# PhantomSDR/PhantomSDR

Measured on AMD Instinct MI355X. Metric: ingest MSamples/s + concurrent audio clients at 2^20-pt FFT, higher is better.
Workload: dtype f32

## Files before the change

phantomsdr_amd/csrc/demod.h:

```cpp
#pragma once
#include <hip/hip_runtime.h>
#include <stdint.h>

#include "butterfly.h"
#include "quantize.h"
#include "types.h"

namespace psdr {



struct DemodArgs {
    const cf *spec;
    size_t spec_stride;
    SpecLayout lay;
    int is_real;
    int n;
    int nframes;
    int max_batch;
    unsigned long long first_frame_num;
    const ClientParams *clients;
    const cf *Wn;
    int nstages;
    int radix[PSDR_MAX_STAGES];
    const int4 *stage_tab;
    cf *ypost;
    float *pwr;
    cf *gscratch;
    int lds_mode;
    float *audio;
    int *nan_flags;
    float *real_prev;
    cf *bb_tail;
    cf *bb_last;
    int slots;
    unsigned *ssb_mark;
    unsigned mark_epoch;
    int replay;
    const int4 *notch_man;
    const int4 *notch_auto;
};
__device__ __forceinline__ bool not_finite(float v) { return !(fabsf(v) <= 3.402823466e38f); }

__device__ __forceinline__ bool flip_frame(unsigned long long frame_num, int m_idx, int is_real) {
    return (frame_num % 2 == 1) && ((m_idx % 2 == 0 && !is_real) || (m_idx % 2 == 1 && is_real));
}
__device__ __forceinline__ float frame_sign(const DemodArgs &a, const ClientParams &cp, int f) {
    return flip_frame(a.first_frame_num + (unsigned long long)f, cp.m_floor, a.is_real) ? -1.f : 1.f;
}

__device__ __forceinline__ void wave_lds_sync() { asm volatile("s_waitcnt lgkmcnt(0)" ::: "memory"); }
__device__ __forceinline__ float wave_sum(float v) {
#pragma unroll
    for (int d = 32; d > 0; d >>= 1) v += __shfl_xor(v, d, 64);
    return v;
}
__device__ __forceinline__ cf *stage_twiddles(const DemodArgs &a, unsigned char *smem, int n) {
    cf *Wn = reinterpret_cast<cf *>(smem);
    for (int i = threadIdx.x; i < n; i += blockDim.x) Wn[i] = a.Wn[i];
    __syncthreads();
    return Wn;
}
__device__ __forceinline__ bool wave_chain(int nact, int F, int K, int &ci, int &f0, int &f1) {
// ... 298 lines not shown
        t = x[1], x[1] = x[3], x[3] = t;
        t = x[2], x[2] = x[6], x[6] = t;
        t = x[5], x[5] = x[7], x[7] = t;
    } else {
        static_assert(R == 10, "butterflies with literal roots: 5, 8, 9, 10");
        idft5(x[0], x[2], x[4], x[6], x[8]);
        idft5(x[1], x[3], x[5], x[7], x[9]);
        const cf w1 = make_float2(0.80901699437494742410f, 0.58778525229247312917f);
        const cf w2 = make_float2(0.30901699437494742410f, 0.95105651629515357212f);
        const cf w3 = make_float2(-0.30901699437494742410f, 0.95105651629515357212f);
        const cf w4 = make_float2(-0.80901699437494742410f, 0.58778525229247312917f);
        cf o1, o2, o3, o4;
        cmul_pair(o1, x[3], w1, o2, x[5], w2);
        cmul_pair(o3, x[7], w3, o4, x[9], w4);
        const cf e0 = x[0], e1 = x[2], e2 = x[4], e3 = x[6], e4 = x[8], o0 = x[1];
        x[0] = cadd(e0, o0), x[5] = csub(e0, o0);
        x[1] = cadd(e1, o1), x[6] = csub(e1, o1);
        x[2] = cadd(e2, o2), x[7] = csub(e2, o2);
        x[3] = cadd(e3, o3), x[8] = csub(e3, o3);
        x[4] = cadd(e4, o4), x[9] = csub(e4, o4);
    }
}

template <int N, int R, int PP>
__device__ __forceinline__ void idft_stage_fixed(cf *buf, const cf *Wn, int lane) {
    constexpr int TLEN = N / R, ROUNDS = (TLEN + 63) / 64, STEP = N / (PP * R);
    constexpr bool RAGGED = (TLEN % 64) != 0;
    cf x[ROUNDS][R];
    int jo[ROUNDS];
#pragma unroll
    for (int rr = 0; rr < ROUNDS; rr++) {
        const int i = lane + 64 * rr;
        if (!RAGGED || rr + 1 < ROUNDS || i < TLEN) {
            const int k = PP == 1 ? 0 : i % PP;
            jo[rr] = (i - k) * R + k;
            x[rr][0] = buf[i];
#pragma unroll
            for (int q = 1; q < R; q++) {
                const cf v = buf[i + q * TLEN];
                if (PP > 1)
                    x[rr][q] = cmul(v, Wn[q * k * STEP]);
                else
                    x[rr][q] = v;
            }
        }
    }
    asm volatile("" ::: "memory");
#pragma unroll
    for (int rr = 0; rr < ROUNDS; rr++) {
        const int i = lane + 64 * rr;
        if (!RAGGED || rr + 1 < ROUNDS || i < TLEN) {
            cf *o = buf + jo[rr];
            idft_bfly<R>(x[rr]);
#pragma unroll
            for (int s = 0; s < R; s++) o[s * PP] = x[rr][s];
        }
    }
}

template <int N>
__device__ __forceinline__ void idft_load_slice(const DemodArgs &a, const ClientParams &cp, const Notches &nz, int f, int lane, cf (&sv)[(N + 63) / 64]) {
    const int len = cp.r - cp.l;
    const cf *S = a.spec + (size_t)f * a.spec_stride;
#pragma unroll
    for (int u = 0; u < (N + 63) / 64; u++) {
        const int t = lane + 64 * u;
        sv[u] = t < len && !notched(nz, cp, t) ? S[a.lay.pos(cp.l + t)] : make_float2(0.f, 0.f);
    }
}
template <int N, int HO>
__device__ __forceinline__ void idft_slice_offsets(const DemodArgs &a, const ClientParams &cp, int lane, unsigned (&so)[HO]) {
    const int len = cp.r - cp.l;
#pragma unroll
    for (int u = 0; u < HO; u++) {
        const int t = lane + 64 * u;
        so[u] = t < len ? (unsigned)a.lay.pos(cp.l + t) : 0u;
    }
}
template <int N, int HO, bool NZ = true>
__device__ __forceinline__ void idft_load_slice_at(const DemodArgs &a, const ClientParams &cp, const Notches &nz, int f, const unsigned (&so)[HO], int lane, cf (&sv)[(N + 63) / 64]) {
    const int len = cp.r - cp.l;
    const cf *S = a.spec + (size_t)f * a.spec_stride;
#pragma unroll
    for (int u = 0; u < (N + 63) / 64; u++) {
        const int t = lane + 64 * u;
        const bool in = t < len && !(NZ && notched(nz, cp, t));
        if (u < HO)
            sv[u] = in ? S[so[u]] : make_float2(0.f, 0.f);
        else
            sv[u] = in ? S[a.lay.pos(cp.l + t)] : make_float2(0.f, 0.f);
    }
}
template <int N, int R0, int R1, int R2>
__device__ __forceinline__ float idft_slice_fixed(const ClientParams &cp, const cf (&sv)[(N + 63) / 64], cf *buf, const cf *Wn, int lane);
template <int N, int R0, int R1, int R2>
__device__ __forceinline__ float idft_item_fixed(const DemodArgs &a, const ClientParams &cp, int f, cf *buf, const cf *Wn, int lane) {
    cf sv[(N + 63) / 64];
    idft_load_slice<N>(a, cp, notch_load(a, cp.slot), f, lane, sv);
    return idft_slice_fixed<N, R0, R1, R2>(cp, sv, buf, Wn, lane);
}
template <int N, int R0, int R1, int R2>
__device__ __forceinline__ float idft_slice_fixed(const ClientParams &cp, const cf (&sv)[(N + 63) / 64], cf *buf, const cf *Wn, int lane) {
    const int len = cp.r - cp.l;
    const int m = cp.m_floor - cp.l;
    constexpr int NR = (N + 63) / 64;
#pragma unroll
    for (int u = 0; u < NR; u++) {
        const int i = lane + 64 * u;
        if (i < N) buf[i] = make_float2(0.f, 0.f);
    }
    asm volatile("" ::: "memory");
    float pw = 0.f;
#pragma unroll
    for (int u = 0; u < NR; u++) {
        const int t = lane + 64 * u;
        if (t < len) {
            const cf v = sv[u];
            pw += fmaf(v.x, v.x, v.y * v.y);
            if (cp.mode < 2) {
                const int idx = cp.mode == 0 ? t - m : m - t;
                if (idx == 0 || idx == N / 2) {
                    buf[idx] = make_float2(v.x, 0.f);
                } else if (idx > 0 && idx < N / 2) {
                    buf[idx] = v;
                    buf[N - idx] = make_float2(v.x, -v.y);
                }
            } else {
                if (t >= m && t < m + N / 2) buf[t - m] = v;
                if (t >= m - N / 2 + 1 && t < m) buf[N - m + t] = v;
            }
        }
    }
    pw = wave_sum(pw);
    wave_lds_sync();
    idft_stage_fixed<N, R0, 1>(buf, Wn, lane);
    wave_lds_sync();
    idft_stage_fixed<N, R1, R0>(buf, Wn, lane);
    wave_lds_sync();
    if constexpr (R2 > 1) {
        idft_stage_fixed<N, R2, R0 * R1>(buf, Wn, lane);
        wave_lds_sync();
    }
    return pw;
}

template <int N, int R0, int R1, int R2>
#ifndef PSDR_IDFT_WPE
#define PSDR_IDFT_WPE 5
#endif
__global__ __launch_bounds__(256, PSDR_IDFT_WPE) void k_demod_idft_fixed(DemodArgs a, int nact) {
    static_assert(R0 * R1 * R2 == N, "plan");
    extern __shared__ __attribute__((aligned(16))) unsigned char smem[];
    const int lane = threadIdx.x & 63, wv = threadIdx.x >> 6;
    cf *Wn = stage_twiddles(a, smem, N);
    int ci, f, f1;
    if (!wave_chain(nact, a.nframes, 1, ci, f, f1)) return;
    const ClientParams cp = wave_uniform(a.clients[ci]);
    cf *buf = Wn + N + (size_t)wv * N;

    const float pw = idft_item_fixed<N, R0, R1, R2>(a, cp, f, buf, Wn, lane);
    if (lane == 0) a.pwr[(size_t)cp.slot * a.max_batch + f] = pw;
    constexpr int NR = (N + 63) / 64;
    const float sg = frame_sign(a, cp, f);
// ... 124 lines not shown
    const size_t srow = (size_t)cp.slot;
    if (cp.mode >= 2 || a.ssb_mark[srow] != a.mark_epoch) return;
    const cf *yp = a.ypost + (srow * a.max_batch) * n;
    const SlotState st = slot_state(a, cp, h);
    int g = -1;
    for (int f = 0; f < a.nframes; f++) {
        const cf *y = yp + (size_t)f * n;
        float *out = a.audio + (srow * a.max_batch + f) * h;
        int s_nan = 0;
        for (int j = tid; j < h; j += NT) {
            const float prev = (g < 0) ? st.rp_old[j] : yp[(size_t)g * n + h + j].x;
            const float v = y[j].x + prev;
            out[j] = v;
            if (isnan(v)) s_nan = 1;
        }
        const int dropped = __any(s_nan);
        if (tid == 0) a.nan_flags[srow * a.max_batch + f] = dropped ? 1 : 0;
        if (!dropped) g = f;
    }
    for (int j = tid; j < h; j += NT) st.rp_new[j] = (g < 0) ? st.rp_old[j] : yp[(size_t)g * n + h + j].x;
}


template <int N, int R0, int R1, int R2>
__global__ __launch_bounds__(256, N <= 512 ? PSDR_IDFT_WPE : PSDR_IDFT_WPE - 1) void k_demod_chain_fixed(DemodArgs a, int nact, int K) {
    static_assert(R0 * R1 * R2 == N, "plan");
    extern __shared__ __attribute__((aligned(16))) unsigned char smem[];
    constexpr int h = N / 2, NH = (h + 63) / 64;
    const int lane_ = threadIdx.x & 63, wv = threadIdx.x >> 6;
    cf *Wn = stage_twiddles(a, smem, N);
    const int F = a.nframes;
    int ci, f0, f1;
    if (!wave_chain(nact, F, K, ci, f0, f1)) return;
    ClientParams cp = a.clients[ci];
    if (a.replay && (cp.mode >= 2 || a.ssb_mark[cp.slot] != a.mark_epoch)) return;
    cp = wave_uniform(cp);
    cf *buf = Wn + N + (size_t)wv * N;
    const size_t srow = (size_t)cp.slot;
    const SlotState st = slot_state(a, cp, h);
    const bool ssb = cp.mode < 2;
    cf tail[NH];
    cf blast = make_float2(0.f, 0.f);
    const int fs = f0 == 0 ? 0 : (f0 - (cp.mode == 3 ? 2 : 1) > 0 ? f0 - (cp.mode == 3 ? 2 : 1) : 0);
#pragma unroll
    for (int u = 0; u < NH; u++) {
        const int j = lane_ + 64 * u;
        tail[u] = make_float2(0.f, 0.f);
        if (fs == 0 && j < h) tail[u] = ssb ? make_float2(st.rp_old[j], 0.f) : st.bt_old[j];
    }
    if (fs == 0 && cp.mode == 3) blast = a.bb_last[st.row_old];
    int bad = 0;
    if (ssb) {
#pragma unroll
        for (int u = 0; u < NH; u++) bad |= not_finite(tail[u].x) ? 1 : 0;
    }
    int f = fs;
#ifndef PSDR_DEMOD_PREFETCH
#define PSDR_DEMOD_PREFETCH 0
#endif
    constexpr int NR = (N + 63) / 64;
    cf svn[NR];
    int fpre = -1;
    constexpr int HO = NR < 3 ? NR : (N <= 512 ? 3 : 6);
    unsigned so[HO];
    idft_slice_offsets<N, HO>(a, cp, lane_, so);
    const Notches nz = notch_load(a, cp.slot);
    while (f < f1) {
        const bool emit = f >= f0;
        const int lane = opaque_lane(lane_);
        float pw;
        if (PSDR_DEMOD_PREFETCH && (N <= 512 || PSDR_DEMOD_PREFETCH > 1)) {
            cf sv[NR];
            if (f == fpre) {
#pragma unroll
                for (int u = 0; u < NR; u++) sv[u] = svn[u];
            } else {
                idft_load_slice_at<N, HO>(a, cp, nz, f, so, lane, sv);
            }
            if (f + 1 < f1) {
                idft_load_slice_at<N, HO>(a, cp, nz, f + 1, so, lane, svn);
                fpre = f + 1;
            }
            pw = idft_slice_fixed<N, R0, R1, R2>(cp, sv, buf, Wn, lane);
        } else {
            cf sv[NR];
            idft_load_slice_at<N, HO>(a, cp, nz, f, so, lane, sv);
            pw = idft_slice_fixed<N, R0, R1, R2>(cp, sv, buf, Wn, lane);
        }
        if (emit && lane == 0) a.pwr[srow * a.max_batch + f] = pw;
        const float sg = frame_sign(a, cp, f);
        float *out = a.audio + (srow * a.max_batch + f) * h;
        const bool last = (f == F - 1);
        int s_nan = 0;
        cf carry = blast;
        cf yv[NH], yn[NH];
        if (cp.mode == 0) {
#pragma unroll
            for (int u = 0; u < NH; u++) {
                const int j = lane + 64 * u;
                yv[u] = yn[u] = make_float2(0.f, 0.f);
                if (j < h) {
                    yv[u].x = __fmul_rn(buf[j].x, sg);
                    yn[u].x = __fmul_rn(buf[h + j].x, sg);
                }
            }
        } else if (cp.mode == 1) {
#pragma unroll
            for (int u = 0; u < NH; u++) {
                const int j = lane + 64 * u;
                yv[u] = yn[u] = make_float2(0.f, 0.f);
                if (j < h) {
                    yv[u].x = __fmul_rn(buf[N - 1 - j].x, sg);
                    yn[u].x = __fmul_rn(buf[N - 1 - h - j].x, sg);
                }
            }
        } else {
#pragma unroll
            for (int u = 0; u < NH; u++) {
                const int j = lane + 64 * u;
                yv[u] = yn[u] = make_float2(0.f, 0.f);
                if (j < h) {
                    const cf v0 = buf[j], v1 = buf[h + j];
                    yv[u] = make_float2(__fmul_rn(v0.x, sg), __fmul_rn(v0.y, sg));
                    yn[u] = make_float2(__fmul_rn(v1.x, sg), __fmul_rn(v1.y, sg));
                }
            }
        }
#pragma unroll
        for (int u = 0; u < NH; u++) {
            const int j = lane + 64 * u;
            const bool ok = j < h;
            const cf y = yv[u], ynext = yn[u];
            float v = 0.f;
            cf b = make_float2(0.f, 0.f);
            if (ssb) {
                v = __fadd_rn(y.x, tail[u].x);
            } else {
                b = make_float2(__fadd_rn(y.x, tail[u].x), __fadd_rn(y.y, tail[u].y));
                if (cp.mode == 2) {
                    v = sqrtf(fmaf(b.x, b.x, b.y * b.y));
                } else {
                    cf pr = make_float2(__shfl_up(b.x, 1, 64), __shfl_up(b.y, 1, 64));
                    if (lane == 0) pr = carry;
                    const float re = fmaf(b.x, pr.x, b.y * pr.y);
                    const float im = fmaf(b.x, -pr.y, b.y * pr.x);
                    v = atan2f(im, re);
                    carry = make_float2(__shfl(b.x, 63, 64), __shfl(b.y, 63, 64));
                    if (u == (h - 1) / 64) blast = make_float2(__shfl(b.x, (h - 1) & 63, 64), __shfl(b.y, (h - 1) & 63, 64));
// ... 2 lines not shown
            if (ok && isnan(v)) s_nan = 1;
            if (ok && emit) {
                out[j] = v;
                if (last && !ssb) {
                    st.bt_new[j] = ynext;
                    st.rp_new[j] = st.rp_old[j];
                    if (j == h - 1) a.bb_last[st.row_new] = b;
                }
            }
            if (!ssb) tail[u] = ynext;
        }
        const int any_nan = __any(s_nan);
        if (ssb) {
#pragma unroll
            for (int u = 0; u < NH; u++) bad |= (not_finite(yv[u].x) || not_finite(yn[u].x)) ? 1 : 0;
            if (!emit) {
                if (any_nan && f > 0) {
                    f--;
                    wave_lds_sync();
                    continue;
                }
#pragma unroll
                for (int u = 0; u < NH; u++) {
                    const int j = lane + 64 * u;
                    tail[u] = yn[u];
                    if (any_nan && j < h) tail[u] = make_float2(st.rp_old[j], 0.f);
                }
                f = f0;
                wave_lds_sync();
                continue;
            }
#pragma unroll
            for (int u = 0; u < NH; u++) {
                const int j = lane + 64 * u;
                if (!any_nan) tail[u] = yn[u];
                if (last && j < h) {
                    st.rp_new[j] = tail[u].x;
                    st.bt_new[j] = st.bt_old[j];
                }
            }
            if (last && lane == 0) a.bb_last[st.row_new] = a.bb_last[st.row_old];
        }
        if (emit && lane == 0) a.nan_flags[srow * a.max_batch + f] = any_nan ? 1 : 0;
        wave_lds_sync();
        f++;
    }
    if (ssb && !a.replay && __any(bad) && lane_ == 0) a.ssb_mark[srow] = a.mark_epoch;
}


template <int N, int R0, int R1, int R2, bool NZ>
__device__ __forceinline__ void demod_chain_iq_body(const DemodArgs &a, int nact, int K, cf *iq) {
    static_assert(R0 * R1 * R2 == N, "plan");
    extern __shared__ __attribute__((aligned(16))) unsigned char smem[];
    constexpr int h = N / 2, NH = (h + 63) / 64;
    const int lane_ = threadIdx.x & 63, wv = threadIdx.x >> 6;
    cf *Wn = stage_twiddles(a, smem, N);
    const int F = a.nframes;
    int ci, f0, f1;
    if (!wave_chain(nact, F, K, ci, f0, f1)) return;
    const ClientParams cp = wave_uniform(a.clients[ci]);
    cf *buf = Wn + N + (size_t)wv * N;
    const size_t srow = (size_t)cp.slot;
    const SlotState st = slot_state(a, cp, h);
    const int fs = f0 == 0 ? 0 : f0 - 1;
    cf tail[NH];
#pragma unroll
    for (int u = 0; u < NH; u++) {
        const int j = lane_ + 64 * u;
        tail[u] = make_float2(0.f, 0.f);
        if (fs == 0 && j < h) tail[u] = st.bt_old[j];
    }
    constexpr int NR = (N + 63) / 64;
    constexpr int HO = NR < 3 ? NR : (N <= 512 ? 3 : 6);
    unsigned so[HO];
    idft_slice_offsets<N, HO>(a, cp, lane_, so);
    for (int f = fs; f < f1; f++) {
        const bool emit = f >= f0;
        const int lane = opaque_lane(lane_);
        Notches nz{};
        if constexpr (NZ) nz = notch_load_frame(a, cp.slot);
        cf sv[NR];
        idft_load_slice_at<N, HO, NZ>(a, cp, nz, f, so, lane, sv);
        const float pw = idft_slice_fixed<N, R0, R1, R2>(cp, sv, buf, Wn, lane);
        if (emit && lane == 0) a.pwr[srow * a.max_batch + f] = pw;
        const float sg = frame_sign(a, cp, f);
        cf *out = iq + (srow * a.max_batch + f) * h;
        const bool last = (f == F - 1);
        int s_nan = 0;
#pragma unroll
        for (int u = 0; u < NH; u++) {
            const int j = lane + 64 * u;
            if (j < h) {
                const cf v0 = buf[j], v1 = buf[h + j];
                const cf y = make_float2(__fmul_rn(v0.x, sg), __fmul_rn(v0.y, sg));
                const cf ynext = make_float2(__fmul_rn(v1.x, sg), __fmul_rn(v1.y, sg));
                const cf b = make_float2(__fadd_rn(y.x, tail[u].x), __fadd_rn(y.y, tail[u].y));
                if (isnan(b.x) || isnan(b.y)) s_nan = 1;
                if (emit) {
                    out[j] = b;
                    if (last) {
                        st.bt_new[j] = ynext;
                        st.rp_new[j] = st.rp_old[j];
                        if (j == h - 1) a.bb_last[st.row_new] = b;
                    }
                }
                tail[u] = ynext;
// ... 89 lines not shown
    idft_slice_offsets<N, HO>(a, cp, lane_, so);
    const int m = cp.m_floor - cp.l;
    cf cC[NH];
#pragma unroll
    for (int u = 0; u < NH; u++) cC[u] = make_float2(0.f, 0.f);
    for (int it = 2 * fs; it < 2 * f1; it++) {
        const int f = it >> 1, pass = it & 1;
        const bool emit = f >= f0;
        const float sg = frame_sign(a, cp, f);
        float *out = a.audio + (srow * a.max_batch + f) * h;
        const bool last = (f == F - 1);
        {
            const int lane = opaque_lane(lane_);
            const Notches nz = notch_load_frame(a, cp.slot);
            cf sv[NR];
            idft_load_slice_at<N, HO>(a, cp, nz, f, so, lane, sv);
            if (pass == 0) {
#pragma unroll
                for (int u = 0; u < NR; u++) {
                    const int d = lane + 64 * u - m;
                    if (d < -sa.cutoff || d >= sa.cutoff) sv[u] = make_float2(0.f, 0.f);
                }
            }
            const float pw = idft_slice_fixed<N, R0, R1, R2>(cp, sv, buf, Wn, lane);
            if (pass == 0) {
#pragma unroll
                for (int u = 0; u < NH; u++) {
                    const int j = lane + 64 * u;
                    cC[u] = make_float2(0.f, 0.f);
                    if (j < h) {
                        const cf v0 = buf[j], v1 = buf[h + j];
                        const cf ct = ctail[j];
                        cC[u] = make_float2(__fadd_rn(__fmul_rn(v0.x, sg), ct.x), __fadd_rn(__fmul_rn(v0.y, sg), ct.y));
                        ctail[j] = make_float2(__fmul_rn(v1.x, sg), __fmul_rn(v1.y, sg));
                    }
                }
            } else {
                if (emit && lane == 0) a.pwr[srow * a.max_batch + f] = pw;
                int s_nan = 0;
                float lvl = 0.f;
                cf lag = make_float2(0.f, 0.f), ccarry = make_float2(0.f, 0.f);
#pragma unroll
                for (int u = 0; u < NH; u++) {
                    const int j = lane + 64 * u;
                    const cf c = cC[u];
                    cf pr = make_float2(__shfl_up(c.x, 1, 64), __shfl_up(c.y, 1, 64));
                    if (lane == 0) pr = ccarry;
// ... 191 lines not shown
        const cf t = ft_rot(64u * (unsigned)u * fc.step);
        wu[u] = make_float2(__int_as_float(__builtin_amdgcn_readfirstlane(__float_as_int(t.x))),
                            __int_as_float(__builtin_amdgcn_readfirstlane(__float_as_int(t.y))));
    }
#endif
    constexpr int NR = (N + 63) / 64;
    constexpr int HO = NR < 3 ? NR : (N <= 512 ? 3 : 6);
    unsigned so[HO];
    idft_slice_offsets<N, HO>(a, cw, lane_, so);
    const Notches nz = notch_load(a, cp.slot);
    for (int f = fs; f < f1; f++) {
        const bool emit = f >= f0;
        const int lane = opaque_lane(lane_);
        cf sv[NR];
        idft_load_slice_at<N, HO>(a, cw, nz, f, so, lane, sv);
        float pw = 0.f;
#pragma unroll
        for (int u = 0; u < NR; u++) {
            const int t = lane + 64 * u;
            if (t < cw.r - cw.l) pw += fmaf(sv[u].x, sv[u].x, sv[u].y * sv[u].y);
            if (t < t0 || t >= t1) sv[u] = make_float2(0.f, 0.f);
        }
        pw = wave_sum(pw);
        idft_slice_fixed<N, R0, R1, R2>(cw, sv, buf, Wn, lane);
        if (emit && lane == 0) a.pwr[srow * a.max_batch + f] = pw;
        const float sg = frame_sign(a, cp, f);
        const bool last = (f == F - 1);
        const unsigned phl = fc.phi0 + ((unsigned)f * (unsigned)h + (unsigned)lane) * fc.step;
        const cf w0 = ft_rot(phl);
        int s_nan = 0;
#pragma unroll
        for (int u = 0; u < NH; u++) {
            const int j = lane + 64 * u;
            if (j < h) {
                const cf v0 = buf[j], v1 = buf[h + j];
                const cf y = make_float2(__fmul_rn(v0.x, sg), __fmul_rn(v0.y, sg));
                const cf ynext = make_float2(__fmul_rn(v1.x, sg), __fmul_rn(v1.y, sg));
                const cf b = make_float2(__fadd_rn(y.x, tail[u].x), __fadd_rn(y.y, tail[u].y));
#if PSDR_FT_ROTATOR_DIRECT
                const cf w = ft_w(phl, fc.step, u);
#else
                const cf w = u == 0 ? w0 : ft_cmul(w0, wu[u]);
#endif
                if constexpr (SSB) {
                    const float v = __fmul_rn(2.f, __fmaf_rn(b.x, w.x, -__fmul_rn(b.y, w.y)));
                    if (isnan(v)) s_nan = 1;
                    if (emit) {
// ... 131 lines not shown
    for (int u = 0; u < NH; u++) cC[u] = make_float2(0.f, 0.f);
    for (int it = 2 * fs; it < 2 * f1; it++) {
        const int f = it >> 1, pass = it & 1;
        const bool emit = f >= f0;
        const float sg = frame_sign(a, cp, f);
        float *out = a.audio + (srow * a.max_batch + f) * h;
        const bool last = (f == F - 1);
        const int lo = pass == 0 ? -sb.sa.cutoff : (upper ? 0 : -N);
        const int hi = pass == 0 ? sb.sa.cutoff : (upper ? N : 1);
        {
            const int lane = opaque_lane(lane_);
            const Notches nz = notch_load_frame(a, cp.slot);
            cf sv[NR];
            idft_load_slice_at<N, HO>(a, cp, nz, f, so, lane, sv);
            float pw = 0.f;
#pragma unroll
            for (int u = 0; u < NR; u++) {
                const int t = lane + 64 * u;
                if (t < len) pw += fmaf(sv[u].x, sv[u].x, sv[u].y * sv[u].y);
                const int d = t - m;
                if (d < lo || d >= hi) sv[u] = make_float2(0.f, 0.f);
            }
            pw = wave_sum(pw);
            idft_slice_fixed<N, R0, R1, R2>(cp, sv, buf, Wn, lane);
            if (pass == 0) {
#pragma unroll
                for (int u = 0; u < NH; u++) {
                    const int j = lane + 64 * u;
                    cC[u] = make_float2(0.f, 0.f);
                    if (j < h) {
                        const cf v0 = buf[j], v1 = buf[h + j];
                        const cf ct = ctail[j];
                        cC[u] = make_float2(__fadd_rn(__fmul_rn(v0.x, sg), ct.x), __fadd_rn(__fmul_rn(v0.y, sg), ct.y));
                        ctail[j] = make_float2(__fmul_rn(v1.x, sg), __fmul_rn(v1.y, sg));
                    }
                }
            } else {
                if (emit && lane == 0) a.pwr[srow * a.max_batch + f] = pw;
                int s_nan = 0;
                float lvl = 0.f;
                cf lag = make_float2(0.f, 0.f), ccarry = make_float2(0.f, 0.f);
#pragma unroll
                for (int u = 0; u < NH; u++) {
                    const int j = lane + 64 * u;
                    const cf c = cC[u];
                    cf pr = make_float2(__shfl_up(c.x, 1, 64), __shfl_up(c.y, 1, 64));
                    if (lane == 0) pr = ccarry;
// ... 215 lines not shown
```

phantomsdr_amd/csrc/demod.hip:

```cpp
#include "ctx.h"
#include "demod.h"
#include "noise.h"
#include "squelch.h"
#include "audiofilter.h"
#include "nr.h"
#include "anb.h"
#include "tone.h"
#include "cw.h"
#include "rtty.h"
#include "psk.h"
#include "fax.h"

template <class Feature>
static int first_use(psdr_ctx *c, Feature &have, const char *msg) {
    if (have) return PSDR_OK;
    HIPCHK(hipSetDevice(c->device));
    Feature fresh;
    if (fresh.alloc(*c)) {
        const std::string why = psdr_last_error();
        return fail(PSDR_ERR_NOMEM, msg, Feature::bytes(*c), why.c_str());
    }
    have = std::move(fresh);
    return PSDR_OK;
}
// ... 491 lines not shown
    case AD_NULL: return fail(PSDR_ERR_INVALID, "null argument");
    case AD_BAD_KIND: return fail(PSDR_ERR_INVALID, "audio filter design: unknown kind %d", kind);
    case AD_BAD_RATE: return fail(PSDR_ERR_INVALID, "audio filter design: audio_rate %g", audio_rate);
    case AD_BAD_F0: return fail(PSDR_ERR_INVALID, "audio filter design: f0 %g outside (0, %g)", f0, audio_rate / 2);
    case AD_BAD_Q: return fail(PSDR_ERR_INVALID, "audio filter design: q %g", q);
    case AD_REFUSED: return fail(PSDR_ERR_INVALID, "audio filter design: kind %d at f0 %g, q %g, rate %g gives a section psdr_client_set_audio_filter refuses", kind, f0, q, audio_rate);
    }
    return PSDR_OK;
}
extern "C" int psdr_debug_notch_ptrs(psdr_ctx *c, const void *out[5]) {
    if (!c || !out) return fail(PSDR_ERR_INVALID, "null argument");
    std::lock_guard<std::mutex> lk(c->mtx);
    out[0] = c->notch.tab.get(), out[1] = c->notch.acc.get(), out[2] = c->notch.cnt.get();
    out[3] = c->dbg_notch_man, out[4] = c->dbg_notch_auto;
    return PSDR_OK;
}

template <class... X>
struct ChainFamily {
    void (*k360)(DemodArgs, int, int, X...);
    void (*k720)(DemodArgs, int, int, X...);
};
static const ChainFamily<> CHAIN_FIXED{k_demod_chain_fixed<360, 8, 9, 5>, k_demod_chain_fixed<720, 8, 9, 10>};
static const ChainFamily<cf *> CHAIN_IQ{k_demod_chain_iq<360, 8, 9, 5>, k_demod_chain_iq<720, 8, 9, 10>};
static const ChainFamily<cf *> CHAIN_IQ_NZ{k_demod_chain_iq_nz<360, 8, 9, 5>, k_demod_chain_iq_nz<720, 8, 9, 10>};
static const ChainFamily<SamArgs> CHAIN_SAM{k_demod_chain_sam<360, 8, 9, 5>, k_demod_chain_sam<720, 8, 9, 10>};
static const ChainFamily<FtArgs> CHAIN_FT_SSB{k_demod_chain_ft<360, 8, 9, 5, true>, k_demod_chain_ft<720, 8, 9, 10, true>};
static const ChainFamily<FtArgs> CHAIN_FT_IQ{k_demod_chain_ft<360, 8, 9, 5, false>, k_demod_chain_ft<720, 8, 9, 10, false>};
static const ChainFamily<SbArgs> CHAIN_SBSAM{k_demod_chain_sbsam<360, 8, 9, 5>, k_demod_chain_sbsam<720, 8, 9, 10>};
static int chain_k(const psdr_ctx *c, int cnt, int nframes) {
    if (c->demod_chain_k > 0) return c->demod_chain_k;
    int K = cnt >= 256 && (unsigned)cnt * (unsigned)((nframes + 15) / 16) >= 8192u ? 16 : 8;
    while (K > 4 && (unsigned)cnt * (unsigned)((nframes + K - 1) / K) < 1024u) K >>= 1;
    return K;
}
template <class... X>
static hipError_t launch_chain(psdr_ctx *c, const ChainFamily<X...> &fam, DemodArgs aa, int cnt, int K, unsigned W360, size_t wave_lds, X... extra) {
    if (K <= 0) K = chain_k(c, cnt, aa.nframes);
    const unsigned W = c->idft_kind == IDFT_FIXED360 ? W360 : 1u;
    const unsigned items = (unsigned)cnt * (unsigned)((aa.nframes + K - 1) / K);
    const size_t lds = (size_t)(1 + W) * c->n * sizeof(cf) + W * wave_lds;
    void *args[] = {&aa, &cnt, &K, &extra...};
    return hipLaunchKernel((const void *)(c->idft_kind == IDFT_FIXED360 ? fam.k360 : fam.k720), dim3((items + W - 1) / W), dim3(64 * W), args, lds, c->side);
}
template <class... X>
static hipError_t launch_ola(psdr_ctx *c, void (*k)(DemodArgs, int, X...), DemodArgs aa, int cnt, X... extra) {
// ... 121 lines not shown
    }
    for (size_t slot : b.rtty.zero) {
        HIPCHK(hipMemsetAsync(c->rtty.state + slot, 0, sizeof(RttyState), c->side));
        HIPCHK(hipMemsetAsync(c->rtty.text + slot * (size_t)RTTY_TEXT, 0, RTTY_TEXT, c->side));
    }
    for (size_t slot : b.psk.zero) {
        HIPCHK(hipMemsetAsync(c->psk.state + slot, 0, sizeof(PskState), c->side));
        HIPCHK(hipMemsetAsync(c->psk.text + slot * (size_t)PSK_TEXT, 0, PSK_TEXT, c->side));
    }
    for (size_t slot : b.fax.zero) HIPCHK(hipMemsetAsync(c->fax.state + slot, 0, sizeof(FaxState), c->side));
    for (size_t slot : b.nf.zero) {
        HIPCHK(hipMemsetAsync(c->noise.acc + slot * (size_t)c->n, 0, (size_t)c->n * sizeof(float), c->side));
        HIPCHK(hipMemsetAsync(c->noise.state + slot, 0, sizeof(NoiseState), c->side));
    }
    c->out_set ^= 1;
    c->d_audio = c->audio_pool[c->out_set], c->d_pwr = c->pwr_pool[c->out_set], c->d_nan = c->nan_pool[c->out_set];
    c->d_iq = b.iq_rows, c->d_car = b.car_rows, c->d_sq = b.sq_rows, c->d_nf = b.nf_rows;
    PSDRCHK(fetch_guard_wait(c, c->side, c->guard_audio[c->out_set]));
    c->guard_audio[c->out_set] = nullptr;
    if (c->post_on && c->post_direct && c->chain_seq >= 2 && c->pc_s[0] && c->side != c->stream)
        HIPCHK(hipStreamWaitEvent(c->side, c->pc.ev[1][(c->chain_seq - 2) % psdr_ctx::PC_SETS], 0));
    for (int i = 0; i < p.ncopies; i++)
        HIPCHK(hipMemcpyAsync(b.d_ring + p.copies[i].off, b.h_ring + p.copies[i].off, p.copies[i].bytes, hipMemcpyHostToDevice, c->side));
    if (p.ntssb > 0 && !c->ft) return fail(PSDR_ERR_STATE, "tuned USB / LSB clients without their tails");
    if (p.nsb > 0 && (!c->sb || !c->sam)) return fail(PSDR_ERR_STATE, "sideband SAM clients without their tails");
    const size_t tail_bytes = ((size_t)c->n / 2) * sizeof(cf);
    for (size_t slot : p.det_zero) PSDRCHK(notch_zero(c, slot));
    for (size_t off : p.car_zero) HIPCHK(hipMemsetAsync(c->sam.car_tail + off, 0, tail_bytes, c->side));
    for (size_t off : p.ft_zero) HIPCHK(hipMemsetAsync(c->ft.tail + off, 0, tail_bytes, c->side));
    for (size_t off : p.sb_zero) HIPCHK(hipMemsetAsync(c->sb.tail + off, 0, tail_bytes, c->side));
    if (b.sq.any()) HIPCHK(c->squelch.tab.upload(b.ring, (size_t)(b.sq.nsq + b.sq.ncopy), c->side));
    if (b.nf.any()) HIPCHK(c->noise.tab.upload(b.ring, (size_t)b.nf.n, c->side));
    if (b.af.any()) HIPCHK(c->af.tab.upload(b.ring, (size_t)b.af.n, c->side));
    if (b.nr.any()) HIPCHK(c->nr.tab.upload(b.ring, (size_t)b.nr.n, c->side));
    if (b.anb.any()) HIPCHK(c->anb.tab.upload(b.ring, (size_t)b.anb.n, c->side));
    if (b.tone.any()) HIPCHK(c->tone.tab.upload(b.ring, (size_t)(b.tone.n + b.tone.ncopy), c->side));
    if (b.cw.any()) HIPCHK(c->cw.tab.upload(b.ring, (size_t)b.cw.n, c->side));
    if (b.rtty.any()) HIPCHK(c->rtty.tab.upload(b.ring, (size_t)b.rtty.n, c->side));
    if (b.psk.any()) HIPCHK(c->psk.tab.upload(b.ring, (size_t)b.psk.n, c->side));
    if (b.fax.any()) HIPCHK(c->fax.tab.upload(b.ring, (size_t)b.fax.n, c->side));
    return PSDR_OK;
}

static bool fixed_plan(const psdr_ctx *c) { return c->idft_kind == IDFT_FIXED360 || c->idft_kind == IDFT_FIXED720; }
static int launch_idft(psdr_ctx *c, const DemodArgs &aa, int cnt) {
    const unsigned items = (unsigned)cnt * (unsigned)aa.nframes;
// ... 4 lines not shown
        const size_t lds = (size_t)(1 + W) * c->n * sizeof(cf);
        if (c->idft_kind == IDFT_FIXED360)
            hipLaunchKernelGGL((k_demod_idft_fixed<360, 8, 9, 5>), dim3((items + W - 1) / W), dim3(64 * W), lds,
                               c->side, aa, cnt);
        else
            hipLaunchKernelGGL((k_demod_idft_fixed<720, 8, 9, 10>), dim3((items + W - 1) / W), dim3(64 * W), lds,
                               c->side, aa, cnt);
        break;
    }
    case IDFT_WAVE: {
        const size_t lds = (size_t)(2 * PSDR_IDFT_WAVES + 1) * c->n * sizeof(cf);
        hipLaunchKernelGGL(k_demod_idft_wave, dim3((items + PSDR_IDFT_WAVES - 1) / PSDR_IDFT_WAVES),
                           dim3(64 * PSDR_IDFT_WAVES), lds, c->side, aa, cnt);
        break;
    }
    default:
        if (c->idft_lds > 64 * 1024 && c->lds_attr_done.insert((const void *)k_demod_idft).second)
            HIPCHK(hipFuncSetAttribute((const void *)k_demod_idft, hipFuncAttributeMaxDynamicSharedMemorySize, (int)c->idft_lds));
        hipLaunchKernelGGL(k_demod_idft, dim3(cnt, aa.nframes), dim3(c->idft_threads), c->idft_lds, c->side,
                           aa);
    }
    return PSDR_OK;
}
static int launch_plain(psdr_ctx *c, const DemodArgs &a, int nold, bool can_be_nonfinite) {
    bool ola_done = false;
    {
        ProfScope ps(c, K_IDFT, c->side);
        if (fixed_plan(c) && c->demod_chain) {
            HIPCHK(launch_chain(c, CHAIN_FIXED, a, nold, 0, 4u, 0));
            if (can_be_nonfinite) {
                DemodArgs ar = a;
                ar.replay = 1;
                HIPCHK(launch_chain(c, CHAIN_FIXED, ar, nold, a.nframes, 4u, 0));
            }
            ola_done = true;
        } else {
            PSDRCHK(launch_idft(c, a, nold));
        }
        HIPCHK(hipGetLastError());
    }
    if (!ola_done) {
        ProfScope ps(c, K_OLA, c->side);
        HIPCHK(launch_ola(c, k_demod_ola, a, nold));
        if (can_be_nonfinite) hipLaunchKernelGGL(k_demod_ola_seq, dim3(((unsigned)nold + 3) / 4), dim3(256), 0, c->side, a, nold);
        HIPCHK(hipGetLastError());
    }
    return PSDR_OK;
}
template <class Fam, class Ola, class Extra>
static int serve(psdr_ctx *c, const Fam &fam, Ola ola, const DemodArgs &aa, int cnt, unsigned W360, size_t wave_lds, Extra extra) {
    if (fixed_plan(c) && c->demod_chain) {
        ProfScope ps(c, K_IDFT, c->side);
        HIPCHK(launch_chain(c, fam, aa, cnt, 0, W360, wave_lds, extra));
        return PSDR_OK;
    }
    {
        ProfScope ps(c, K_IDFT, c->side);
        PSDRCHK(launch_idft(c, aa, cnt));
        HIPCHK(hipGetLastError());
    }
    ProfScope ps(c, K_OLA, c->side);
    HIPCHK(launch_ola(c, ola, aa, cnt, extra));
    return PSDR_OK;
}
static int launch_lists(psdr_ctx *c, const BatchPlan &b, const DemodArgs &a, bool can_be_nonfinite) {
    const DemodPlan &p = b.p;
    auto of_list = [&](const RingList &l) {
        DemodArgs al = a;
        al.clients = ring_at<ClientParams>(b.d_ring, l.clients);
        return al;
    };
    if (p.nold > 0) PSDRCHK(launch_plain(c, a, p.nold, can_be_nonfinite));
    const size_t tail_bytes = ((size_t)c->n / 2) * sizeof(cf);
    SamArgs sa{};
    if (p.nsam + p.nsb > 0) {
        sa.car_tail = c->sam.car_tail;
        sa.car_rec = c->d_car;
        sa.cutoff = (int)((int64_t)500 * c->n / c->cfg.audio_rate);
        sa.hz_per_rad = (float)((double)c->cfg.audio_rate / (2.0 * M_PI));
    }
    if (p.nsam > 0) PSDRCHK(serve(c, CHAIN_SAM, k_demod_ola_sam, of_list(p.sam), p.nsam, 2u, tail_bytes, sa));
    if (p.niq > 0) PSDRCHK(serve(c, p.iq_notched ? CHAIN_IQ_NZ : CHAIN_IQ, k_demod_ola_iq, of_list(p.iq), p.niq, 4u, 0, c->d_iq));
    FtArgs fa{};
    fa.tail = c->ft.tail;
    fa.iq = c->d_iq;
    if (p.ntssb > 0) {
        fa.ft = ring_at<FtClient>(b.d_ring, p.tssb.side);
        PSDRCHK(serve(c, CHAIN_FT_SSB, k_demod_ola_ft<true>, of_list(p.tssb), p.ntssb, 4u, 0, fa));
    }
    if (p.ntiq > 0) {
        fa.ft = ring_at<FtClient>(b.d_ring, p.tiq.side);
        PSDRCHK(serve(c, CHAIN_FT_IQ, k_demod_ola_ft<false>, of_list(p.tiq), p.ntiq, 4u, 0, fa));
    }
    if (p.nsb > 0) {
        SbArgs sba{};
// ... 210 lines not shown
```

phantomsdr_amd/csrc/demodplan.h:

```cpp
#pragma once
#include <stddef.h>
#include <stdint.h>

#include <algorithm>
#include <cmath>
#include <vector>

#include "../../include/psdr.h"
#include "types.h"

namespace psdr {

struct AfSection {
    float b0 = 0, b1 = 0, b2 = 0, a1 = 0, a2 = 0, pad[3] = {0, 0, 0};
    float P[6][4] = {};
};
static_assert(sizeof(AfSection) == 128, "the device table's layout");

struct FaxEntry {
    int slot, mode, width, K, D, NB, start_blocks, phase_lines, max_lines, wp, R, pad;
    uint64_t Lq, origin0;
    uint32_t inc, tinc[3];
    float rot[2], trot[3][2];
    float s, ratio, shift, nbh;
// ... 116 lines not shown
    int n = 0;
    int nframes = 0;
    bool post_on = false;
    bool have_notch_tab = false;
    bool has_band = false;
    uint32_t band_first = 0, band_count = 0;
};

enum DemodVerdict { DP_OK, DP_BAND_OUTSIDE };
struct RingSpan {
    size_t off = 0, bytes = 0;
};
struct RingList {
    size_t clients = 0, side = 0;
};
struct DemodPlan {
    DemodVerdict verdict = DP_OK;
    int bad_slot = -1, bad_l = 0, bad_r = 0;
    int nold = 0, nsam = 0, ntssb = 0, ntiq = 0, nsb = 0, niq = 0, nact = 0, npaused = 0, ndet = 0, iq_off = 0;
    RingList plain, sam, iq, tssb, tiq, sb, det;
    size_t slot_ci = 0, notch = 0;
    RingSpan copies[5];
    int ncopies = 0;
    std::vector<size_t> car_zero, ft_zero, sb_zero, det_zero;
    bool any_manual = false;
    bool iq_notched = false;
    bool idle() const { return nact + niq + ntiq == 0; }
};

inline DemodPlan demod_plan(AudioSlot *slots, size_t S, uint64_t &demod_seq, const DemodFacts &f, unsigned char *ring_host) {
    DemodPlan p;
    if (f.has_band)
        for (size_t i = 0; i < S; i++) {
            const AudioSlot &s = slots[i];
            if (s.active && !s.paused && s.r > s.l && ((uint32_t)s.l < f.band_first || (uint64_t)s.r > (uint64_t)f.band_first + f.band_count)) {
                p.verdict = DP_BAND_OUTSIDE;
                p.bad_slot = (int)i, p.bad_l = s.l, p.bad_r = s.r;
                return p;
            }
        }
    const size_t h = (size_t)f.n / 2;
    ClientParams *const clients = (ClientParams *)ring_host;
    int *const slot_ci = (int *)(clients + S);
    int *const notch = (int *)(ring_host + notch_ring_off(S));
    ClientParams *const det = (ClientParams *)(ring_host + notch_ring_off(S) + S * NOTCH_ENTRY);
    p.slot_ci = S * sizeof(ClientParams), p.notch = notch_ring_off(S), p.det.clients = p.notch + S * NOTCH_ENTRY;
// ... 65 lines not shown
        AudioSlot &s = slots[q.slot];
        ((ClientParams *)(ring_host + p.tssb.clients))[k] = placed(q, s.mode != PSDR_IQ, s.mode == PSDR_USB);
        FtClient &t = ((FtClient *)(ring_host + p.tssb.side))[k];
        t.step = (uint32_t)std::floor((s.mid - std::floor(s.mid)) * 4294967296.0 / f.n + 0.5);
        t.phi0 = s.ft_phi;
        t.l = q.l, t.r = q.r;
        s.ft_phi += (uint32_t)f.nframes * (uint32_t)(f.n / 2) * t.step;
    };

    int k = 0;
    for (int i : of[CK_PLAIN]) clients[k++] = listed(i);
    for (int i : of[CK_SAM]) clients[k++] = listed(i);
    for (int j = 0; j < p.ntssb; j++, k++) list_tuned(j, clients[k] = listed(of[CK_FT_SSB][j]));
    for (int j = 0; j < p.nsb; j++, k++) {
        const AudioSlot &s = slots[of[CK_SBSAM][j]];
        clients[k] = listed(of[CK_SBSAM][j]);
        ((ClientParams *)(ring_host + p.sb.clients))[j] = placed(clients[k], true, s.sam_sb == PSDR_SAM_UPPER);
        ((SbClient *)(ring_host + p.sb.side))[j] = SbClient{clients[k].l, clients[k].r, s.sam_sb, 0};
    }
    if (f.post_on) {
        std::fill(slot_ci, slot_ci + S, -1);
        for (int j = 0; j < p.nact; j++) slot_ci[clients[j].slot] = j;
    }
    const bool chain = f.post_on && p.nact > 0;
    auto list_paused = [&](const ClientParams &q) {
        slot_ci[q.slot] = p.nact + p.npaused;
        clients[p.nact + p.npaused++] = q;
    };
    if (chain)
        for (int i : of[CK_PAUSED])
            if (slots[i].agc_reset != 2) {
                ClientParams q{};
                q.slot = i, q.state_cur = slots[i].state_cur, q.paused = 1;
                list_paused(q);
            }
    for (int j = 0; j < p.ntiq; j++) {
        const ClientParams q = listed(of[CK_FT_IQ][j]);
        list_tuned(p.ntssb + j, q);
        if (chain && slots[q.slot].agc_reset != 2) list_paused(q);
    }
    if (p.niq > 0) {
        p.iq_off = k = p.nact + p.npaused;
        for (int fresh = 0; fresh < 2; fresh++)
            for (int i : of[CK_IQ])
                if ((slots[i].agc_reset == 2) == (fresh == 1)) {
                    clients[k] = listed(i);
// ... 18 lines not shown
```

Before: 103,000.

## Split plain demod chain into SSB and complex kernels with branchless scatter

Plain-demod clients are partitioned on the host into SSB (USB/LSB) and complex families through a family index uploaded to the device ring. Each family gets its own chain kernel specialisation, so the per-client mode branches become compile-time and only SSB clients are replayed for non-finite recovery. The IDFT stages and output loops also clamp ragged lane indices instead of wrapping loads in conditionals, and the spectrum scatter is made branchless. This adds an extra kernel launch and host-to-device copy when both families are present, and relies on index clamping to stay correct at the ragged edges.

```diff
diff --git a/phantomsdr_amd/csrc/demod.h b/phantomsdr_amd/csrc/demod.h
--- a/phantomsdr_amd/csrc/demod.h
+++ b/phantomsdr_amd/csrc/demod.h
@@ -39,6 +39,7 @@
     int replay;
     const int4 *notch_man;
     const int4 *notch_auto;
+    const int *fam_index;
 };
 __device__ __forceinline__ bool not_finite(float v) { return !(fabsf(v) <= 3.402823466e38f); }
 
@@ -383,7 +384,7 @@
     }
 }
 
-template <int N, int R, int PP>
+template <int N, int R, int PP, bool CLAMP = true>
 __device__ __forceinline__ void idft_stage_fixed(cf *buf, const cf *Wn, int lane) {
     constexpr int TLEN = N / R, ROUNDS = (TLEN + 63) / 64, STEP = N / (PP * R);
     constexpr bool RAGGED = (TLEN % 64) != 0;
@@ -391,28 +392,29 @@
     int jo[ROUNDS];
 #pragma unroll
     for (int rr = 0; rr < ROUNDS; rr++) {
-        const int i = lane + 64 * rr;
-        if (!RAGGED || rr + 1 < ROUNDS || i < TLEN) {
-            const int k = PP == 1 ? 0 : i % PP;
-            jo[rr] = (i - k) * R + k;
-            x[rr][0] = buf[i];
-#pragma unroll
-            for (int q = 1; q < R; q++) {
-                const cf v = buf[i + q * TLEN];
-                if (PP > 1)
-                    x[rr][q] = cmul(v, Wn[q * k * STEP]);
-                else
-                    x[rr][q] = v;
-            }
+        const bool ragged = RAGGED && rr + 1 == ROUNDS;
+        if (!CLAMP && ragged && lane + 64 * rr >= TLEN) continue;
+        const int i = CLAMP && ragged ? min(lane + 64 * rr, TLEN - 1) : lane + 64 * rr;
+        const int k = PP == 1 ? 0 : i % PP;
+        jo[rr] = (i - k) * R + k;
+        x[rr][0] = buf[i];
+#pragma unroll
+        for (int q = 1; q < R; q++) {
+            const cf v = buf[i + q * TLEN];
+            if (PP > 1)
+                x[rr][q] = cmul(v, Wn[q * k * STEP]);
+            else
+                x[rr][q] = v;
         }
     }
     asm volatile("" ::: "memory");
 #pragma unroll
     for (int rr = 0; rr < ROUNDS; rr++) {
-        const int i = lane + 64 * rr;
-        if (!RAGGED || rr + 1 < ROUNDS || i < TLEN) {
-            cf *o = buf + jo[rr];
-            idft_bfly<R>(x[rr]);
+        const bool live = !RAGGED || rr + 1 < ROUNDS || lane + 64 * rr < TLEN;
+        if (!CLAMP && !live) continue;
+        cf *o = buf + jo[rr];
+        idft_bfly<R>(x[rr]);
+        if (live) {
 #pragma unroll
             for (int s = 0; s < R; s++) o[s * PP] = x[rr][s];
         }
@@ -452,7 +454,7 @@
             sv[u] = in ? S[a.lay.pos(cp.l + t)] : make_float2(0.f, 0.f);
     }
 }
-template <int N, int R0, int R1, int R2>
+template <int N, int R0, int R1, int R2, int FAM = 0, bool CLAMP = true>
 __device__ __forceinline__ float idft_slice_fixed(const ClientParams &cp, const cf (&sv)[(N + 63) / 64], cf *buf, const cf *Wn, int lane);
 template <int N, int R0, int R1, int R2>
 __device__ __forceinline__ float idft_item_fixed(const DemodArgs &a, const ClientParams &cp, int f, cf *buf, const cf *Wn, int lane) {
@@ -460,7 +462,7 @@
     idft_load_slice<N>(a, cp, notch_load(a, cp.slot), f, lane, sv);
     return idft_slice_fixed<N, R0, R1, R2>(cp, sv, buf, Wn, lane);
 }
-template <int N, int R0, int R1, int R2>
+template <int N, int R0, int R1, int R2, int FAM, bool CLAMP>
 __device__ __forceinline__ float idft_slice_fixed(const ClientParams &cp, const cf (&sv)[(N + 63) / 64], cf *buf, const cf *Wn, int lane) {
     const int len = cp.r - cp.l;
     const int m = cp.m_floor - cp.l;
@@ -472,34 +474,42 @@
     }
     asm volatile("" ::: "memory");
     float pw = 0.f;
-#pragma unroll
-    for (int u = 0; u < NR; u++) {
-        const int t = lane + 64 * u;
-        if (t < len) {
+    const bool ssb = FAM == 1 || (FAM == 0 && cp.mode < 2);
+    if (ssb) {
+        const int flip = cp.mode == 0 ? 0 : -1;
+#pragma unroll
+        for (int u = 0; u < NR; u++) {
+            const int t = lane + 64 * u;
             const cf v = sv[u];
             pw += fmaf(v.x, v.x, v.y * v.y);
-            if (cp.mode < 2) {
-                const int idx = cp.mode == 0 ? t - m : m - t;
-                if (idx == 0 || idx == N / 2) {
-                    buf[idx] = make_float2(v.x, 0.f);
-                } else if (idx > 0 && idx < N / 2) {
-                    buf[idx] = v;
-                    buf[N - idx] = make_float2(v.x, -v.y);
-                }
-            } else {
-                if (t >= m && t < m + N / 2) buf[t - m] = v;
-                if (t >= m - N / 2 + 1 && t < m) buf[N - m + t] = v;
-            }
+            const int idx = ((t - m) ^ flip) - flip;
+            const bool edge = idx == 0 || idx == N / 2;
+            const int mir = edge ? idx : N - idx;
+            const float im = edge ? 0.f : v.y, mim = edge ? 0.f : -v.y;
+            if (t < len && (unsigned)idx <= (unsigned)(N / 2)) {
+                buf[idx] = make_float2(v.x, im);
+                buf[mir] = make_float2(v.x, mim);
+            }
+        }
+    } else {
+#pragma unroll
+        for (int u = 0; u < NR; u++) {
+            const int t = lane + 64 * u;
+            const cf v = sv[u];
+            pw += fmaf(v.x, v.x, v.y * v.y);
+            const int d = t - m;
+            const int idx = d < 0 ? d + N : d;
+            if (t < len && (unsigned)(d + N / 2 - 1) < (unsigned)(N - 1)) buf[idx] = v;
         }
     }
     pw = wave_sum(pw);
     wave_lds_sync();
-    idft_stage_fixed<N, R0, 1>(buf, Wn, lane);
+    idft_stage_fixed<N, R0, 1, CLAMP>(buf, Wn, lane);
     wave_lds_sync();
-    idft_stage_fixed<N, R1, R0>(buf, Wn, lane);
+    idft_stage_fixed<N, R1, R0, CLAMP>(buf, Wn, lane);
     wave_lds_sync();
     if constexpr (R2 > 1) {
-        idft_stage_fixed<N, R2, R0 * R1>(buf, Wn, lane);
+        idft_stage_fixed<N, R2, R0 * R1, CLAMP>(buf, Wn, lane);
         wave_lds_sync();
     }
     return pw;
@@ -670,31 +680,34 @@
 }
 
 
-template <int N, int R0, int R1, int R2>
-__global__ __launch_bounds__(256, N <= 512 ? PSDR_IDFT_WPE : PSDR_IDFT_WPE - 1) void k_demod_chain_fixed(DemodArgs a, int nact, int K) {
+template <int N, int R0, int R1, int R2, bool SSB>
+__device__ __forceinline__ void demod_chain_fixed_body(const DemodArgs &a, int nact, int K) {
     static_assert(R0 * R1 * R2 == N, "plan");
     extern __shared__ __attribute__((aligned(16))) unsigned char smem[];
     constexpr int h = N / 2, NH = (h + 63) / 64;
+    constexpr bool ssb = SSB;
     const int lane_ = threadIdx.x & 63, wv = threadIdx.x >> 6;
     cf *Wn = stage_twiddles(a, smem, N);
     const int F = a.nframes;
     int ci, f0, f1;
     if (!wave_chain(nact, F, K, ci, f0, f1)) return;
+    if (a.fam_index) ci = a.fam_index[ci];
     ClientParams cp = a.clients[ci];
-    if (a.replay && (cp.mode >= 2 || a.ssb_mark[cp.slot] != a.mark_epoch)) return;
+    if (SSB && a.replay && a.ssb_mark[cp.slot] != a.mark_epoch) return;
     cp = wave_uniform(cp);
     cf *buf = Wn + N + (size_t)wv * N;
     const size_t srow = (size_t)cp.slot;
     const SlotState st = slot_state(a, cp, h);
-    const bool ssb = cp.mode < 2;
     cf tail[NH];
     cf blast = make_float2(0.f, 0.f);
     const int fs = f0 == 0 ? 0 : (f0 - (cp.mode == 3 ? 2 : 1) > 0 ? f0 - (cp.mode == 3 ? 2 : 1) : 0);
+    const bool flips = (cp.m_floor % 2 == 0 && !a.is_real) || (cp.m_floor % 2 == 1 && a.is_real);
+    const unsigned par0 = (unsigned)(a.first_frame_num & 1ull);
 #pragma unroll
     for (int u = 0; u < NH; u++) {
-        const int j = lane_ + 64 * u;
+        const int jc = min(lane_ + 64 * u, h - 1);
         tail[u] = make_float2(0.f, 0.f);
-        if (fs == 0 && j < h) tail[u] = ssb ? make_float2(st.rp_old[j], 0.f) : st.bt_old[j];
+        if (fs == 0) tail[u] = ssb ? make_float2(st.rp_old[jc], 0.f) : st.bt_old[jc];
     }
     if (fs == 0 && cp.mode == 3) blast = a.bb_last[st.row_old];
     int bad = 0;
@@ -729,49 +742,39 @@
                 idft_load_slice_at<N, HO>(a, cp, nz, f + 1, so, lane, svn);
                 fpre = f + 1;
             }
-            pw = idft_slice_fixed<N, R0, R1, R2>(cp, sv, buf, Wn, lane);
+            pw = idft_slice_fixed<N, R0, R1, R2, SSB ? 1 : 2>(cp, sv, buf, Wn, lane);
         } else {
             cf sv[NR];
             idft_load_slice_at<N, HO>(a, cp, nz, f, so, lane, sv);
-            pw = idft_slice_fixed<N, R0, R1, R2>(cp, sv, buf, Wn, lane);
-        }
-        if (emit && lane == 0) a.pwr[srow * a.max_batch + f] = pw;
-        const float sg = frame_sign(a, cp, f);
+            pw = idft_slice_fixed<N, R0, R1, R2, SSB ? 1 : 2>(cp, sv, buf, Wn, lane);
+        }
+        const float sg = (flips && ((par0 + (unsigned)f) & 1u)) ? -1.f : 1.f;
         float *out = a.audio + (srow * a.max_batch + f) * h;
         const bool last = (f == F - 1);
         int s_nan = 0;
         cf carry = blast;
         cf yv[NH], yn[NH];
-        if (cp.mode == 0) {
+        if (SSB && cp.mode == 0) {
 #pragma unroll
             for (int u = 0; u < NH; u++) {
-                const int j = lane + 64 * u;
-                yv[u] = yn[u] = make_float2(0.f, 0.f);
-                if (j < h) {
-                    yv[u].x = __fmul_rn(buf[j].x, sg);
-                    yn[u].x = __fmul_rn(buf[h + j].x, sg);
-                }
-            }
-        } else if (cp.mode == 1) {
+                const int jc = min(lane + 64 * u, h - 1);
+                yv[u] = make_float2(__fmul_rn(buf[jc].x, sg), 0.f);
+                yn[u] = make_float2(__fmul_rn(buf[h + jc].x, sg), 0.f);
+            }
+        } else if (SSB) {
 #pragma unroll
             for (int u = 0; u < NH; u++) {
-                const int j = lane + 64 * u;
-                yv[u] = yn[u] = make_float2(0.f, 0.f);
-                if (j < h) {
-                    yv[u].x = __fmul_rn(buf[N - 1 - j].x, sg);
-                    yn[u].x = __fmul_rn(buf[N - 1 - h - j].x, sg);
-                }
+                const int jc = min(lane + 64 * u, h - 1);
+                yv[u] = make_float2(__fmul_rn(buf[N - 1 - jc].x, sg), 0.f);
+                yn[u] = make_float2(__fmul_rn(buf[N - 1 - h - jc].x, sg), 0.f);
             }
         } else {
 #pragma unroll
             for (int u = 0; u < NH; u++) {
-                const int j = lane + 64 * u;
-                yv[u] = yn[u] = make_float2(0.f, 0.f);
-                if (j < h) {
-                    const cf v0 = buf[j], v1 = buf[h + j];
-                    yv[u] = make_float2(__fmul_rn(v0.x, sg), __fmul_rn(v0.y, sg));
-                    yn[u] = make_float2(__fmul_rn(v1.x, sg), __fmul_rn(v1.y, sg));
-                }
+                const int jc = min(lane + 64 * u, h - 1);
+                const cf v0 = buf[jc], v1 = buf[h + jc];
+                yv[u] = make_float2(__fmul_rn(v0.x, sg), __fmul_rn(v0.y, sg));
+                yn[u] = make_float2(__fmul_rn(v1.x, sg), __fmul_rn(v1.y, sg));
             }
         }
 #pragma unroll
@@ -820,9 +823,9 @@
                 }
 #pragma unroll
                 for (int u = 0; u < NH; u++) {
-                    const int j = lane + 64 * u;
+                    const int jc = min(lane + 64 * u, h - 1);
                     tail[u] = yn[u];
-                    if (any_nan && j < h) tail[u] = make_float2(st.rp_old[j], 0.f);
+                    if (any_nan) tail[u] = make_float2(st.rp_old[jc], 0.f);
                 }
                 f = f0;
                 wave_lds_sync();
@@ -839,11 +842,22 @@
             }
             if (last && lane == 0) a.bb_last[st.row_new] = a.bb_last[st.row_old];
         }
-        if (emit && lane == 0) a.nan_flags[srow * a.max_batch + f] = any_nan ? 1 : 0;
+        if (emit && lane == 0) {
+            a.pwr[srow * a.max_batch + f] = pw;
+            a.nan_flags[srow * a.max_batch + f] = any_nan ? 1 : 0;
+        }
         wave_lds_sync();
         f++;
     }
     if (ssb && !a.replay && __any(bad) && lane_ == 0) a.ssb_mark[srow] = a.mark_epoch;
+}
+template <int N, int R0, int R1, int R2>
+__global__ __launch_bounds__(256, N <= 512 ? PSDR_IDFT_WPE : PSDR_IDFT_WPE - 1) void k_demod_chain_fixed(DemodArgs a, int nact, int K) {
+    demod_chain_fixed_body<N, R0, R1, R2, true>(a, nact, K);
+}
+template <int N, int R0, int R1, int R2>
+__global__ __launch_bounds__(256, N <= 512 ? PSDR_IDFT_WPE : PSDR_IDFT_WPE - 1) void k_demod_chain_fixed_cplx(DemodArgs a, int nact, int K) {
+    demod_chain_fixed_body<N, R0, R1, R2, false>(a, nact, K);
 }
 
 
@@ -880,7 +894,7 @@
         if constexpr (NZ) nz = notch_load_frame(a, cp.slot);
         cf sv[NR];
         idft_load_slice_at<N, HO, NZ>(a, cp, nz, f, so, lane, sv);
-        const float pw = idft_slice_fixed<N, R0, R1, R2>(cp, sv, buf, Wn, lane);
+        const float pw = idft_slice_fixed<N, R0, R1, R2, 2>(cp, sv, buf, Wn, lane);
         if (emit && lane == 0) a.pwr[srow * a.max_batch + f] = pw;
         const float sg = frame_sign(a, cp, f);
         cf *out = iq + (srow * a.max_batch + f) * h;
@@ -1016,7 +1030,7 @@
                     if (d < -sa.cutoff || d >= sa.cutoff) sv[u] = make_float2(0.f, 0.f);
                 }
             }
-            const float pw = idft_slice_fixed<N, R0, R1, R2>(cp, sv, buf, Wn, lane);
+            const float pw = idft_slice_fixed<N, R0, R1, R2, 2>(cp, sv, buf, Wn, lane);
             if (pass == 0) {
 #pragma unroll
                 for (int u = 0; u < NH; u++) {
@@ -1254,7 +1268,7 @@
             if (t < t0 || t >= t1) sv[u] = make_float2(0.f, 0.f);
         }
         pw = wave_sum(pw);
-        idft_slice_fixed<N, R0, R1, R2>(cw, sv, buf, Wn, lane);
+        idft_slice_fixed<N, R0, R1, R2, 2, false>(cw, sv, buf, Wn, lane);
         if (emit && lane == 0) a.pwr[srow * a.max_batch + f] = pw;
         const float sg = frame_sign(a, cp, f);
         const bool last = (f == F - 1);
@@ -1432,7 +1446,7 @@
                 if (d < lo || d >= hi) sv[u] = make_float2(0.f, 0.f);
             }
             pw = wave_sum(pw);
-            idft_slice_fixed<N, R0, R1, R2>(cp, sv, buf, Wn, lane);
+            idft_slice_fixed<N, R0, R1, R2, 0>(cp, sv, buf, Wn, lane);
             if (pass == 0) {
 #pragma unroll
                 for (int u = 0; u < NH; u++) {
diff --git a/phantomsdr_amd/csrc/demod.hip b/phantomsdr_amd/csrc/demod.hip
--- a/phantomsdr_amd/csrc/demod.hip
+++ b/phantomsdr_amd/csrc/demod.hip
@@ -537,6 +537,7 @@
     void (*k720)(DemodArgs, int, int, X...);
 };
 static const ChainFamily<> CHAIN_FIXED{k_demod_chain_fixed<360, 8, 9, 5>, k_demod_chain_fixed<720, 8, 9, 10>};
+static const ChainFamily<> CHAIN_FIXED_CPLX{k_demod_chain_fixed_cplx<360, 8, 9, 5>, k_demod_chain_fixed_cplx<720, 8, 9, 10>};
 static const ChainFamily<cf *> CHAIN_IQ{k_demod_chain_iq<360, 8, 9, 5>, k_demod_chain_iq<720, 8, 9, 10>};
 static const ChainFamily<cf *> CHAIN_IQ_NZ{k_demod_chain_iq_nz<360, 8, 9, 5>, k_demod_chain_iq_nz<720, 8, 9, 10>};
 static const ChainFamily<SamArgs> CHAIN_SAM{k_demod_chain_sam<360, 8, 9, 5>, k_demod_chain_sam<720, 8, 9, 10>};
@@ -704,6 +705,8 @@
         HIPCHK(hipStreamWaitEvent(c->side, c->pc.ev[1][(c->chain_seq - 2) % psdr_ctx::PC_SETS], 0));
     for (int i = 0; i < p.ncopies; i++)
         HIPCHK(hipMemcpyAsync(b.d_ring + p.copies[i].off, b.h_ring + p.copies[i].off, p.copies[i].bytes, hipMemcpyHostToDevice, c->side));
+    if (p.fam_index.bytes > 0)
+        HIPCHK(hipMemcpyAsync(b.d_ring + p.fam_index.off, b.h_ring + p.fam_index.off, p.fam_index.bytes, hipMemcpyHostToDevice, c->side));
     if (p.ntssb > 0 && !c->ft) return fail(PSDR_ERR_STATE, "tuned USB / LSB clients without their tails");
     if (p.nsb > 0 && (!c->sb || !c->sam)) return fail(PSDR_ERR_STATE, "sideband SAM clients without their tails");
     const size_t tail_bytes = ((size_t)c->n / 2) * sizeof(cf);
@@ -754,16 +757,21 @@
     }
     return PSDR_OK;
 }
-static int launch_plain(psdr_ctx *c, const DemodArgs &a, int nold, bool can_be_nonfinite) {
+static int launch_plain(psdr_ctx *c, const BatchPlan &b, const DemodArgs &a, bool can_be_nonfinite) {
+    const DemodPlan &p = b.p;
+    const int nold = p.nold;
     bool ola_done = false;
     {
         ProfScope ps(c, K_IDFT, c->side);
         if (fixed_plan(c) && c->demod_chain) {
-            HIPCHK(launch_chain(c, CHAIN_FIXED, a, nold, 0, 4u, 0));
-            if (can_be_nonfinite) {
-                DemodArgs ar = a;
-                ar.replay = 1;
-                HIPCHK(launch_chain(c, CHAIN_FIXED, ar, nold, a.nframes, 4u, 0));
+            const int K = chain_k(c, nold, a.nframes);
+            DemodArgs as = a, ac = a;
+            if (p.fam_index.bytes > 0) as.fam_index = ring_at<int>(b.d_ring, p.fam_ssb), ac.fam_index = ring_at<int>(b.d_ring, p.fam_cplx);
+            if (p.nssb > 0) HIPCHK(launch_chain(c, CHAIN_FIXED, as, p.nssb, K, 4u, 0));
+            if (p.ncplx > 0) HIPCHK(launch_chain(c, CHAIN_FIXED_CPLX, ac, p.ncplx, K, 4u, 0));
+            if (can_be_nonfinite && p.nssb > 0) {
+                as.replay = 1;
+                HIPCHK(launch_chain(c, CHAIN_FIXED, as, p.nssb, a.nframes, 4u, 0));
             }
             ola_done = true;
         } else {
@@ -802,7 +810,7 @@
         al.clients = ring_at<ClientParams>(b.d_ring, l.clients);
         return al;
     };
-    if (p.nold > 0) PSDRCHK(launch_plain(c, a, p.nold, can_be_nonfinite));
+    if (p.nold > 0) PSDRCHK(launch_plain(c, b, a, can_be_nonfinite));
     const size_t tail_bytes = ((size_t)c->n / 2) * sizeof(cf);
     SamArgs sa{};
     if (p.nsam + p.nsb > 0) {
diff --git a/phantomsdr_amd/csrc/demodplan.h b/phantomsdr_amd/csrc/demodplan.h
--- a/phantomsdr_amd/csrc/demodplan.h
+++ b/phantomsdr_amd/csrc/demodplan.h
@@ -162,6 +162,9 @@
     size_t slot_ci = 0, notch = 0;
     RingSpan copies[5];
     int ncopies = 0;
+    int nssb = 0, ncplx = 0;
+    RingSpan fam_index;
+    size_t fam_ssb = 0, fam_cplx = 0;
     std::vector<size_t> car_zero, ft_zero, sb_zero, det_zero;
     bool any_manual = false;
     bool iq_notched = false;
@@ -273,6 +276,15 @@
         std::fill(slot_ci, slot_ci + S, -1);
         for (int j = 0; j < p.nact; j++) slot_ci[clients[j].slot] = j;
     }
+    static_assert(sizeof(int) <= sizeof(ClientParams) + sizeof(FtClient) && (sizeof(ClientParams) + sizeof(FtClient)) % sizeof(int) == 0, "the family index fits behind the tuned lists");
+    for (int j = 0; j < p.nold; j++) (clients[j].mode == PSDR_USB || clients[j].mode == PSDR_LSB ? p.nssb : p.ncplx)++;
+    if (p.nssb > 0 && p.ncplx > 0) {
+        p.fam_index = RingSpan{p.sb.clients + (size_t)p.nsb * (sizeof(ClientParams) + sizeof(SbClient)), (size_t)p.nold * sizeof(int)};
+        p.fam_ssb = p.fam_index.off, p.fam_cplx = p.fam_index.off + (size_t)p.nssb * sizeof(int);
+        int *const ix = (int *)(ring_host + p.fam_index.off);
+        int ks = 0, kc = p.nssb;
+        for (int j = 0; j < p.nold; j++) ix[clients[j].mode == PSDR_USB || clients[j].mode == PSDR_LSB ? ks++ : kc++] = j;
+    }
     const bool chain = f.post_on && p.nact > 0;
     auto list_paused = [&](const ClientParams &q) {
         slot_ci[q.slot] = p.nact + p.npaused;
```

Result: no change. 103,000 (median of 2 runs) (+0.0%).
